# Stalfoes/dqn_mgsc_zoo

Hardware: AMD Instinct MI355X
Metric: learner grad-steps/sec at batch=32, 84×84×4 uint8, 1/2/4/8 MI355X (higher is better)
Workload: dtype f32

## Files before the change

dqn_mgsc_zoo_amd/_native.py:

```python

import ctypes
import glob
import hashlib
import os
import threading

_HERE = os.path.dirname(os.path.abspath(__file__))
LIB_PATH = os.environ.get('DQZ_LIB') or os.path.join(_HERE, 'libdqz.so')
HEADER_PATH = os.path.join(os.path.dirname(_HERE), 'include', 'dqz.h')

DQZ_OK = 0
ALGO_DQN = 0
ALGO_DOUBLE = 1
ALGO_PER = 2
NUM_LEAVES = 10
NUM_PHASES = 10
PHASE_NAMES = (
    'conv1_fwd', 'conv2_fwd', 'conv3_fwd', 'fc1_fwd', 'head', 'fc1_dx',
    'conv3_dx+conv2_dx+fc1_dw+conv3_dw+conv2_dw+conv1_dw', 'unused7',
    'unused8', 'update')
FRAME_H = 84
FRAME_W = 84
STACK = 4
FRAME_BYTES = FRAME_H * FRAME_W
# ... 272 lines not shown
    'dqz_qr_forward_slots': (
        _int, [_vp, _vp, ctypes.POINTER(DqzStore), _vp, _int, _int, _vp, _vp]),
    'dqz_qr_act': (
        _int, [_vp, _vp, _vp, _int, ctypes.c_double, ctypes.c_uint64,
               ctypes.c_uint64, _vp, _vp]),
    'dqz_qr_debug_check': (_int, [_int, ctypes.c_uint]),
    'dqz_learner_grad': (
        _int,
        [_vp, ctypes.POINTER(DqzParams), ctypes.POINTER(DqzStore), _vp, _vp,
         _vp, _vp],
    ),
    'dqz_learner_outputs': (_int, [_vp, _vp, _vp, _vp, _vp]),
    'dqz_learner_sync_status': (_int, [_vp, _vp]),
    'dqz_learner_debug_stall': (_int, [_vp, _int, ctypes.c_uint]),
    'dqz_learner_debug_backward': (_int, [_vp, _int, _vp]),
    'dqz_learner_debug_activations': (_int, [_vp, _int] + [_vp] * 10),
    'dqz_per_write_back': (_int, [_vp, _vp, _i64, _vp, ctypes.c_double, _vp, _vp]),
    'dqz_learner_profile': (
        _int,
        [_vp, ctypes.POINTER(DqzParams), ctypes.POINTER(DqzStore), _vp, _vp,
         _int, ctypes.POINTER(ctypes.c_float), _vp],
    ),
    'dqz_forward': (_int, [_vp, _vp, _vp, _int, _vp, _vp]),
    'dqz_forward_slots': (
        _int, [_vp, _vp, ctypes.POINTER(DqzStore), _vp, _int, _int, _vp, _vp]),
    'dqz_act': (
        _int, [_vp, _vp, _vp, _int, ctypes.c_double, ctypes.c_uint64,
               ctypes.c_uint64, _vp, _vp]),
    'dqz_store_put': (
        _int, [ctypes.POINTER(DqzStore), ctypes.POINTER(DqzTransitionPut), _vp,
# ... 159 lines not shown
```

dqn_mgsc_zoo_amd/csrc/bwd.hpp:

```cpp
#pragma once
#include "common.hpp"
#include "conv1.hpp"
#include "fwd.hpp"
#include "head.hpp"
#include "sampling.hpp"

namespace dqz {

struct Fc1BwdArgs {
  const float* dz1;
  const float* y3;
  float *th, *mu, *nu;
  int64_t w_off;
  Rms rms;
  int B;
  float* dy3;
  const float *w3, *w2;
  float *w3p, *w2p;
};

__device__ __forceinline__ int w3p_src(int i) {
  const int j = i & 3, kq = (i >> 2) & 3, n = (i >> 4) & 15, w = (i >> 8) & 3, r = i >> 10;
  const int tp = r % 9, nq = r / 9;
  return ((8 - tp) * C3CI + 16 * nq + n) * C3CO + 16 * w + 4 * j + kq;
// ... 296 lines not shown
      const float4 v = wp[tp * 256];
      wr[4 * tp] = v.x;
      wr[4 * tp + 1] = v.y;
      wr[4 * tp + 2] = v.z;
      wr[4 * tp + 3] = v.w;
    }
#pragma unroll
    for (int k = 0; k < 2; ++k) {
      const int q = min((t >> 2) + 64 * k, 99), ah = q / 10, cw = q % 10;
      ym4[k] = *reinterpret_cast<const float4*>(a.y1 + ((int64_t)b * C1M + (2 * ah + ph) * C1O + 2 * cw + pw) * C1CO +
                                                16 * hh + 4 * (t & 3));
    }
  }
  const float4* src = reinterpret_cast<const float4*>(a.dy2 + (int64_t)b * (C2M * C2CO));
  constexpr int NW4 = 121 * 16;
  if constexpr (WAIT) a.sync.wait(b);
  float4 r[8];
#pragma unroll
  for (int q = 0; q < 8; ++q) {
    const int i = min(t + 256 * q, NW4 - 1);
    const int pix = i >> 4, oh = pix / 11 - 1, ow = pix % 11 - 1;
    const bool in = oh >= 0 && oh < C2O && ow >= 0 && ow < C2O;
    const int e = (in ? oh * C2O + ow : 0) * 16 + (i & 15);
    float4 v;
    if constexpr (WAIT)
      v = load_sc1_f4(src, C2M * C2CO * 4, e);
    else
      v = src[e];
    r[q] = in ? v : make_float4(0.f, 0.f, 0.f, 0.f);
  }
  __builtin_amdgcn_sched_barrier(0);
#pragma unroll
  for (int q = 0; q < 8; ++q) {
    const int i = t + 256 * q;
    if (i < NW4) {
      const int pix = i >> 4;
      float* d = s_win + (pix / 11) * C2X_RS + (pix % 11) * C2X_S + win64_ch((i & 15) * 4);
      d[0] = r[q].x;
      d[1] = r[q].y;
      d[2] = r[q].z;
      d[3] = r[q].w;
    }
  }
  __syncthreads();
  DQZ_STAMP(7, 1);
  constexpr int MT = 6;
  int base[MT];
#pragma unroll
  for (int m = 0; m < MT; ++m) {
    const int p = min(16 * m + n, 99);
    base[m] = (p / 10) * C2X_RS + (p % 10) * C2X_S + win64_ch(16 * w) + kq;
  }
  f32x4 acc[MT];
#pragma unroll
  for (int m = 0; m < MT; ++m) acc[m] = f32x4{0.f, 0.f, 0.f, 0.f};
  float last[4] = {0.f, 0.f, 0.f, 0.f};
#pragma unroll
  for (int kk = 0; kk < 16; ++kk) {
    const int tp = kk >> 2;
// ... 1 lines not shown
#pragma unroll
    for (int m = 0; m < MT; ++m) acc[m] = mfma4(s_win[base[m] + off], wr[kk], acc[m]);
    {
#pragma unroll
      for (int e = 0; e < 4; ++e)
        last[e] = __fmaf_rn(s_win[9 * C2X_RS + (6 + e) * C2X_S + win64_ch(16 * w) + kq + off], wr[kk], last[e]);
    }
  }
  {
#pragma unroll
    for (int e = 0; e < 4; ++e) {
      last[e] += __shfl_xor(last[e], 16, 64);
      last[e] += __shfl_xor(last[e], 32, 64);
    }
  }
  __syncthreads();
  DQZ_STAMP(7, 2);
  float* s_red = s_win;
#pragma unroll
  for (int m = 0; m < MT; ++m)
#pragma unroll
    for (int rr = 0; rr < 4; ++rr) s_red[w * 1792 + (16 * m + 4 * kq + rr) * 16 + n] = acc[m][rr];
  if (kq == 0) {
#pragma unroll
    for (int e = 0; e < 4; ++e) s_red[w * 1792 + (96 + e) * 16 + n] = last[e];
  }
  __syncthreads();
#pragma unroll
  for (int k = 0; k < 2; ++k) {
    const int q = (t >> 2) + 64 * k;
// ... 4 lines not shown
      for (int e = 0; e < 4; ++e)
        v[e] = (s_red[i + e] + s_red[1792 + i + e]) + (s_red[3584 + i + e] + s_red[5376 + i + e]);
      v[0] = ym4[k].x > 0.f ? v[0] : 0.f;
      v[1] = ym4[k].y > 0.f ? v[1] : 0.f;
      v[2] = ym4[k].z > 0.f ? v[2] : 0.f;
      v[3] = ym4[k].w > 0.f ? v[3] : 0.f;
      float* slab = a.dy1 + (int64_t)b * C1M * C1CO;
      const int off = (((2 * ah + ph) * C1O + 2 * cw + pw) * C1CO + 16 * hh + 4 * (t & 3)) * 4;
      if constexpr (PUB)
        store_sc1_f4(slab, C1M * C1CO * 4, off, v);
      else
        *reinterpret_cast<f32x4*>(reinterpret_cast<char*>(slab) + off) = v;
    }
  }
  if constexpr (PUB) a.sync1.arrive(b);
}

constexpr int C2V_WIN = 9 * C2W_RS;

__device__ __forceinline__ void conv2_bwd_dw_split(const Conv2BwdArgs& a, float* s_win, int b, int kh, int ch) {
  const int t = threadIdx.x, lane = t & 63, w = t >> 6;
  const int n = lane & 15, kq = lane >> 4;
  constexpr int NV4 = 9 * C1O * C1CO / 4;
  float4 r[6];
  {
    const float4* src = reinterpret_cast<const float4*>(a.y1 + (int64_t)b * (C1M * C1CO));
#pragma unroll
    for (int q = 0; q < 6; ++q) {
      const int i = min(t + 256 * q, NV4 - 1);
      const int oh = i / (C1O * 8), rem = i % (C1O * 8);
// ... 7 lines not shown
    pb[kk] = (p / C2O) * C2W_RS + (2 * (p % C2O) + w) * C2W_S + n;
  }
  f32x4 acc[2][2];
#pragma unroll
  for (int mt = 0; mt < 2; ++mt)
#pragma unroll
    for (int ct = 0; ct < 2; ++ct) acc[mt][ct] = f32x4{0.f, 0.f, 0.f, 0.f};
#pragma unroll
  for (int q = 0; q < 6; ++q) {
    const int i = t + 256 * q;
    if (i < NV4) {
      const int oh = i / (C1O * 8), rem = i % (C1O * 8), iw = rem >> 3;
      *reinterpret_cast<float4*>(s_win + oh * C2W_RS + iw * C2W_S + (rem & 7) * 4) = r[q];
    }
  }
  a.sync.wait(b);
  float dr[21][2];
#pragma unroll
  for (int kk = 0; kk < 21; ++kk) {
    const int p = 4 * kk + kq;
#pragma unroll
    for (int ct = 0; ct < 2; ++ct) {
      const float* gp = a.dy2 + ((int64_t)b * C2M + min(p, C2M - 1)) * C2CO + 32 * ch + 16 * ct + n;
      const float v = __hip_atomic_load(gp, __ATOMIC_RELAXED, __HIP_MEMORY_SCOPE_AGENT);
      dr[kk][ct] = p < C2M ? v : 0.f;
    }
  }
  __syncthreads();
  DQZ_STAMP(13, 1);
#pragma unroll
  for (int kk = 0; kk < 21; ++kk)
#pragma unroll
    for (int mt = 0; mt < 2; ++mt) {
      const float av = s_win[pb[kk] + 16 * mt];
#pragma unroll
      for (int ct = 0; ct < 2; ++ct) acc[mt][ct] = mfma4(dr[kk][ct], av, acc[mt][ct]);
    }
  float sb[2] = {0.f, 0.f};
#pragma unroll
  for (int ct = 0; ct < 2; ++ct)
#pragma unroll
    for (int kk = 0; kk < 21; ++kk) sb[ct] += dr[kk][ct];
  float* slab = a.part + (int64_t)b * (C2KK + 1) * C2CO;
#pragma unroll
  for (int mt = 0; mt < 2; ++mt)
#pragma unroll
    for (int ct = 0; ct < 2; ++ct)
      *reinterpret_cast<f32x4*>(slab + ((kh * C2K + w) * C2CI + 16 * mt + n) * C2CO + 32 * ch + 16 * ct + 4 * kq) =
          acc[mt][ct];
  if (kh == 0 && w == 0) {
#pragma unroll
    for (int ct = 0; ct < 2; ++ct) {
// ... 341 lines not shown
```

dqn_mgsc_zoo_amd/csrc/common.hpp:

```cpp
#pragma once
#include <hip/hip_runtime.h>

#include <cstdarg>
#include <cstdint>
#include <cstdio>
#include <string>

#include "dqz.h"

namespace dqz {

typedef float f32x4 __attribute__((ext_vector_type(4)));

#define DQZ_STR(x) #x
#define DQZ_XSTR(x) DQZ_STR(x)
typedef float f32x16 __attribute__((ext_vector_type(16)));

#ifdef DQZ_STEP_TU
#define DQZ_STEP_KERNEL __global__
#define DQZ_OTHER_KERNEL template <int = 0> __global__
#else
#define DQZ_STEP_KERNEL template <int = 0> __global__
#define DQZ_OTHER_KERNEL __global__
#endif
// ... 100 lines not shown
    const float w = 2.f * u * (-lr) * rs3 * (d2 - c1 * g * (g - m));
    nu = w;
    sq += u * u;
    s1 += gq * w;
  }
  __device__ __forceinline__ float meta2(float g, float m0, float v0, float j, float& sq) const {
    const float m = c1 * g + decay * m0;
    const float v = c1 * (g * g) + decay * v0;
    const float u = (-lr) * (g * rsqrtf(v - m * m + eps));
    sq += u * u;
    return -2.f * u * j;
  }
};

#ifdef DQZ_TRACE
constexpr int TRACE_KERNELS = 20, TRACE_BLOCKS = 4096, TRACE_SLOTS = 4;
static __device__ unsigned long long g_dqz_trace[TRACE_KERNELS * TRACE_BLOCKS * TRACE_SLOTS];
#define DQZ_STAMP(kid, slot)                                                                              \
  do {                                                                                                    \
    if (threadIdx.x == 0) {                                                                               \
      const unsigned bl_ = blockIdx.x + gridDim.x * (blockIdx.y + gridDim.y * blockIdx.z);                \
      if (bl_ < (unsigned)dqz::TRACE_BLOCKS)                                                              \
        dqz::g_dqz_trace[((kid) * dqz::TRACE_BLOCKS + bl_) * dqz::TRACE_SLOTS + (slot)] =                \
            __builtin_amdgcn_s_memrealtime();                                                             \
    }                                                                                                     \
  } while (0)
#else
#define DQZ_STAMP(kid, slot) \
  do {                       \
  } while (0)
#endif
// ... 71 lines not shown

inline dim3 xcd_grid(int J, int nsamp) { return dim3((unsigned)(J * ((nsamp + 7) / 8) * 8)); }

struct Handoff {
  static constexpr int kStride = 64;
  int* cnt;
  int* ack;
  int* err;
  int need, consumers;
  unsigned spin_max = 1u << 24;
  __device__ __forceinline__ void arrive(int b) const {
    asm volatile("s_waitcnt vmcnt(0)" ::: "memory");
    __syncthreads();
    if (threadIdx.x == 0) __hip_atomic_fetch_add(cnt + b * kStride, 1, __ATOMIC_RELAXED, __HIP_MEMORY_SCOPE_AGENT);
  }
  __device__ __forceinline__ void wait(int b) const {
    if (threadIdx.x == 0) {
      unsigned spins = 0;
      while (__hip_atomic_load(cnt + b * kStride, __ATOMIC_RELAXED, __HIP_MEMORY_SCOPE_AGENT) < need) {
        __builtin_amdgcn_s_sleep(4);
        if (++spins > spin_max) {
          __hip_atomic_fetch_or(err, 1, __ATOMIC_RELAXED, __HIP_MEMORY_SCOPE_AGENT);
          break;
        }
      }
      if (__hip_atomic_fetch_add(ack + b * kStride, 1, __ATOMIC_RELAXED, __HIP_MEMORY_SCOPE_AGENT) == consumers - 1) {
        __hip_atomic_store(cnt + b * kStride, 0, __ATOMIC_RELAXED, __HIP_MEMORY_SCOPE_AGENT);
        __hip_atomic_store(ack + b * kStride, 0, __ATOMIC_RELAXED, __HIP_MEMORY_SCOPE_AGENT);
      }
    }
    __syncthreads();
  }
};

__device__ __forceinline__ float4 load_sc1_f4(const float4* base, int bytes, int e) {
  typedef unsigned u32x4 __attribute__((ext_vector_type(4)));
  const __amdgpu_buffer_rsrc_t r = __builtin_amdgcn_make_buffer_rsrc((void*)base, 0, bytes, 0x00020000);
  return __builtin_bit_cast(float4, __builtin_amdgcn_raw_buffer_load_b128(r, e * 16, 0, 16));
}

__device__ __forceinline__ float load_sc1_f1(const float* base, int bytes, int e) {
  const __amdgpu_buffer_rsrc_t r = __builtin_amdgcn_make_buffer_rsrc((void*)base, 0, bytes, 0x00020000);
  return __builtin_bit_cast(float, __builtin_amdgcn_raw_buffer_load_b32(r, e * 4, 0, 16));
}

__device__ __forceinline__ void store_sc1_f4(float* base, int bytes, int off, f32x4 v) {
  typedef unsigned u32x4 __attribute__((ext_vector_type(4)));
  const __amdgpu_buffer_rsrc_t r = __builtin_amdgcn_make_buffer_rsrc((void*)base, 0, bytes, 0x00020000);
// ... 26 lines not shown
```

dqn_mgsc_zoo_amd/csrc/conv1.hpp:

```cpp
#pragma once
#include "common.hpp"
#include "sampling.hpp"

namespace dqz {

struct Conv1Src {
  const uint8_t* frames;
  const int32_t* fidx;
  const int32_t* slots;
  const uint8_t* states;
  int fused;
  union {
    UniformDraw draw;
    SoftmaxDraw sm;
    PerSampleArgs per;
    SoftmaxDrawExact smx;
  };
  const int32_t* action = nullptr;
  const float* reward = nullptr;
  const float* discount = nullptr;
  float4* rec = nullptr;
  uint8_t* xout = nullptr;
};

// ... 272 lines not shown
  const int row0 = rb * C1S * C1_ROWS;
  constexpr int QPC = C1_PLANE / 16;
  uint4 v = make_uint4(0u, 0u, 0u, 0u);
  const int tid = threadIdx.x;
  const int cl = tid / QPC, pj = tid % QPC;
  if constexpr (PRE) {
    v = vpre;
  } else {
    const int slot = a.src.slots[b];
    const int32_t* fr = a.src.fidx + (int64_t)slot * 8 + a.which * 4 + 2 * ch;
    const int fa = fr[0], fb = fr[1];
    const int f = cl == 0 ? fa : fb;
    if (tid < 2 * QPC && f >= 0)
      v = reinterpret_cast<const uint4*>(a.src.frames + (int64_t)f * FB + row0 * FW)[pj];
  }
  a.sync1.wait(b);
  const float* dyb = a.dy1 + ((int64_t)b * C1M + rb * C1_POS) * C1CO;
  const int co = tid & 31, c0 = tid >> 5;
  float dv[2][8];
#pragma unroll
  for (int it = 0; it < 2; ++it) {
    const int c = c0 + 8 * it, oh = c / 3, ow0 = 8 * (c % 3);
#pragma unroll
    for (int j = 0; j < 8; ++j)
      dv[it][j] = (c < 15 && ow0 + j < C1O)
                      ? load_sc1_f1(dyb, C1_POS * C1CO * 4, (oh * C1O + ow0 + j) * C1CO + co) : 0.f;
  }
  if (tid < 2 * QPC) store_bytes_as_bf16(s_in + cl * C1_PLANE + pj * 16, v);
#pragma unroll
  for (int it = 0; it < 2; ++it) {
    const int c = c0 + 8 * it;
    unsigned pk[3][4];
    float sb = 0.f;
#pragma unroll
    for (int j = 0; j < 8; j += 2) {
      unsigned h0, m0, l0, h1, m1, l1;
      split3_bf16(dv[it][j], h0, m0, l0);
      split3_bf16(dv[it][j + 1], h1, m1, l1);
      pk[0][j / 2] = h0 | (h1 << 16);
      pk[1][j / 2] = m0 | (m1 << 16);
      pk[2][j / 2] = l0 | (l1 << 16);
      sb += dv[it][j];
      sb += dv[it][j + 1];
    }
#pragma unroll
    for (int q = 0; q < 3; ++q)
      *reinterpret_cast<uint4*>(s_dt + (q * C1CO + co) * C1H_TLD + 8 * c) =
          make_uint4(pk[q][0], pk[q][1], pk[q][2], pk[q][3]);
    s_bp[c * C1CO + co] = sb;
  }
  __syncthreads();
  DQZ_STAMP(8, 1);
  const int lane = tid & 63, wave = tid >> 6;
  const int h = lane >> 5, i = lane & 31;
  float* part = a.part + ((int64_t)b * C1_BLOCKS + rb) * (C1KK + 1) * C1CO;
  if (ch == 0 && tid < C1CO) {
    float sb = 0.f;
    for (int c = 0; c < 15; ++c) sb += s_bp[c * C1CO + tid];
    part[C1KK * C1CO + tid] = sb;
  }
  const int kh = 2 * wave + (i >> 4), kw = (i >> 1) & 7, cp = i & 1;
  const uint16_t* pb = s_in + cp * C1_PLANE + kh * FW + kw;
  const uint16_t* pa = s_dt + i * C1H_TLD + 8 * h;
  f32x16 acc = {};
#pragma unroll
  for (int s = 0; s < 8; ++s) {
    constexpr int R = 4 * FW;
    const int o0 = (2 * s) / 3 * R + 32 * ((2 * s) % 3);
    const int o1 = 2 * s + 1 < 15 ? (2 * s + 1) / 3 * R + 32 * ((2 * s + 1) % 3) : 0;
    const uint16_t* px = pb + (h ? o1 : o0);
    unsigned xp[4];
#pragma unroll
    for (int j = 0; j < 8; j += 2) xp[j / 2] = (unsigned)px[4 * j] | ((unsigned)px[4 * j + 4] << 16);
    const bf16x8 xb = __builtin_bit_cast(bf16x8, make_uint4(xp[0], xp[1], xp[2], xp[3]));
#pragma unroll
    for (int q = 0; q < 3; ++q) {
      const bf16x8 dq = __builtin_bit_cast(bf16x8, *reinterpret_cast<const uint4*>(pa + q * C1CO * C1H_TLD + 16 * s));
      acc = __builtin_amdgcn_mfma_f32_32x32x16_bf16(dq, xb, acc, 0, 0, 0);
    }
  }
  {
    const int row = (2 * wave + (i >> 4)) * 32 + ((i >> 1) & 7) * 4 + 2 * ch + (i & 1);
#pragma unroll
    for (int q = 0; q < 4; ++q)
      *reinterpret_cast<f32x4*>(part + row * C1CO + 8 * q + 4 * h) =
          f32x4{div255(acc[4 * q]), div255(acc[4 * q + 1]), div255(acc[4 * q + 2]), div255(acc[4 * q + 3])};
  }
  DQZ_STAMP(8, 3);
}

__device__ __forceinline__ void conv1_dw_half(const Conv1DwArgs& a, float* smem, int rb, int ch, int b) {
  DQZ_STAMP(8, 0);
  conv1_dw_body<false>(a, smem, make_uint4(0u, 0u, 0u, 0u), rb, ch, b);
}

// ... 2 lines not shown
```

dqn_mgsc_zoo_amd/csrc/fwd.hpp:

```cpp
#pragma once
#include "common.hpp"
#include "conv1.hpp"

namespace dqz {


__device__ __forceinline__ f32x4 mfma4(float a, float b, f32x4 c) {
  return __builtin_amdgcn_mfma_f32_16x16x4f32(a, b, c, 0, 0, 0);
}

__device__ __forceinline__ int red_idx(int row, int col) { return row * 16 + 16 * (row >> 2) + col; }

__device__ __forceinline__ int epi_row(int i) {
  return ((i >> 6) << 4) + (int)((0xFBAE9DC873261540ull >> (4 * ((i >> 2) & 15))) & 15);
}
constexpr int epi_range(int rows) { return (rows + 15) / 16 * 64; }
constexpr int red_rows(int rows) { return rows * 16 + 16 * ((rows + 3) / 4); }

struct LayerFwdArgs {
  const float* in;
  NetZ nz;
  int64_t w_off, b_off;
  int B, Z;
  int linear;
// ... 8 lines not shown
template <bool WAIT, bool PUB>
__device__ __forceinline__ void conv2_fwd_body(const LayerFwdArgs& a, float* s_in, const SampleJob sj) {
  DQZ_STAMP(1, 0);
  const int nq = sj.job, b = sj.s % a.B, z = sj.s / a.B;
  const int t = threadIdx.x, lane = t & 63, w = t >> 6;
  const int n = lane & 15, kq = lane >> 4;
  const float* W = a.nz.p[z] + a.w_off;
  const float bv = a.nz.p[z][a.b_off + 16 * nq + (t & 15)];
  const float4 bias4 = PUB ? *reinterpret_cast<const float4*>(a.nz.p[z] + a.b_off + 16 * nq + 4 * (t & 3))
                           : make_float4(0.f, 0.f, 0.f, 0.f);
  float wr[32];
#pragma unroll
  for (int kk = 0; kk < 32; ++kk) wr[kk] = W[(w * 128 + 4 * kk + kq) * C2CO + 16 * nq + n];
  const float4* src = reinterpret_cast<const float4*>(a.in + ((int64_t)z * a.B + b) * (C1M * C1CO));
  constexpr int NQ4 = C1M * C1CO / 4;
  if constexpr (WAIT) a.wait.wait(sj.s);
  float4 r[13];
#pragma unroll
  for (int q = 0; q < 13; ++q) {
    if constexpr (WAIT)
      r[q] = load_sc1_f4(src, NQ4 * 16, min(t + 256 * q, NQ4 - 1));
    else
      r[q] = src[min(t + 256 * q, NQ4 - 1)];
  }
  __builtin_amdgcn_sched_barrier(0);
#pragma unroll
  for (int q = 0; q < 13; ++q) {
    const int i = t + 256 * q;
    if (i < NQ4) {
      const int pix = i >> 3, ci = (i & 7) * 4;
      float* d = s_in + (pix / C1O) * C2L_RS + (pix % C1O) * C2L_S + ci;
      d[0] = r[q].x;
      d[1] = r[q].y;
      d[2] = r[q].z;
      d[3] = r[q].w;
    }
  }
  DQZ_STAMP(1, 1);
  __syncthreads();
  constexpr int MT = 5;
  int base[MT];
#pragma unroll
  for (int m = 0; m < MT; ++m) {
    const int p = min(16 * m + n, C2M - 1);
    base[m] = (2 * (p / C2O) + w) * C2L_RS + 2 * (p % C2O) * C2L_S + kq;
  }
  f32x4 acc[MT];
#pragma unroll
  for (int m = 0; m < MT; ++m) acc[m] = f32x4{0.f, 0.f, 0.f, 0.f};
  float last = 0.f;
  const int blast = (2 * (C2O - 1) + w) * C2L_RS + 2 * (C2O - 1) * C2L_S + kq;
#pragma unroll
  for (int kk = 0; kk < 32; ++kk) {
    const int off = (kk >> 3) * C2L_S + 4 * (kk & 7);
#pragma unroll
    for (int m = 0; m < MT; ++m) acc[m] = mfma4(s_in[base[m] + off], wr[kk], acc[m]);
    last = __fmaf_rn(s_in[blast + off], wr[kk], last);
  }
  DQZ_STAMP(1, 2);
  {
    last += __shfl_xor(last, 16, 64);
    last += __shfl_xor(last, 32, 64);
  }
  __syncthreads();
  float* s_red = s_in;
  constexpr int RW = red_rows(96);
  static_assert(4 * RW <= C2L_WIN, "conv2 partials fit the window");
#pragma unroll
  for (int m = 0; m < MT; ++m)
#pragma unroll
    for (int rr = 0; rr < 4; ++rr) s_red[w * RW + red_idx(16 * m + 4 * kq + rr, n)] = acc[m][rr];
  if (kq == 0) s_red[w * RW + red_idx(C2M - 1, n)] = last;
  __syncthreads();
  float* out = a.out + ((int64_t)z * a.B + b) * (C2M * C2CO) + 16 * nq;
// ... 4 lines not shown
  if constexpr (PUB) {
    for (int i = t; i < epi_range(C2M); i += 256) {
      const int p = epi_row(i), c4 = 4 * (i & 3);
      if (p >= C2M) continue;
      float o[4];
#pragma unroll
      for (int e = 0; e < 4; ++e) {
        const int k = red_idx(p, c4 + e);
        const float bb = e == 0 ? bias4.x : e == 1 ? bias4.y : e == 2 ? bias4.z : bias4.w;
        const float v = ((s_red[k] + s_red[RW + k]) + (s_red[2 * RW + k] + s_red[3 * RW + k])) + bb;
        o[e] = linear ? v : relu(v);
      }
      store_sc1_f4(out, (C2M * C2CO - 16 * nq) * 4, 4 * (p * C2CO + c4), f32x4{o[0], o[1], o[2], o[3]});
    }
    a.pub.arrive(sj.s);
  } else {
    for (int i = t; i < C2M * 16; i += 256) {
      const int k = red_idx(i >> 4, i & 15);
      const float v = ((s_red[k] + s_red[RW + k]) + (s_red[2 * RW + k] + s_red[3 * RW + k])) + bv;
      if (dot)
        dacc += v * dyp[(i >> 4) * C2CO + (i & 15)];
      else
        out[(i >> 4) * C2CO + (i & 15)] = linear ? v : relu(v);
    }
  }
  if (!PUB && dot) {
    __syncthreads();
    const float r = block_sum256(dacc, s_in);
    if (t == 0) a.dot.part[(int64_t)b * META_DOT_SLOTS + a.dot.slot0 + nq] = r;
  }
// ... 4 lines not shown
__device__ __forceinline__ void conv2_fwd8_body(const LayerFwdArgs& a, float* s_in, const SampleJob sj) {
  DQZ_STAMP(1, 0);
  const int rh = sj.job >> 2, nq = sj.job & 3, b = sj.s % a.B, z = sj.s / a.B;
  const int oh0 = rh * C2F_ROWS0, npos = (rh ? C2O - C2F_ROWS0 : C2F_ROWS0) * C2O;
  const int ih0 = C2S * oh0, nrows = C2S * (npos / C2O - 1) + C2K;
  const int t = threadIdx.x, lane = t & 63, w = t >> 6;
  const int n = lane & 15, kq = lane >> 4;
  const float* W = a.nz.p[z] + a.w_off;
  const float4 bias4 = *reinterpret_cast<const float4*>(a.nz.p[z] + a.b_off + 16 * nq + 4 * (t & 3));
  float wr[32];
#pragma unroll
  for (int kk = 0; kk < 32; ++kk) wr[kk] = W[(w * 128 + 4 * kk + kq) * C2CO + 16 * nq + n];
  const float4* src = reinterpret_cast<const float4*>(a.in + ((int64_t)z * a.B + b) * (C1M * C1CO)) +
                      ih0 * C1O * (C1CO / 4);
  const int nq4 = nrows * C1O * (C1CO / 4);
  a.wait.wait(sj.s);
  constexpr int NL = (2 * C2F_ROWS0 + 2) * C1O * (C1CO / 4) / 256;
  float4 r[NL + 1];
#pragma unroll
  for (int q = 0; q <= NL; ++q) r[q] = load_sc1_f4(src, nq4 * 16, min(t + 256 * q, nq4 - 1));
  __builtin_amdgcn_sched_barrier(0);
#pragma unroll
  for (int q = 0; q <= NL; ++q) {
    const int i = t + 256 * q;
    if (i < nq4) {
      const int pix = i >> 3, ci = (i & 7) * 4;
      float* d = s_in + (pix / C1O) * C2L_RS + (pix % C1O) * C2L_S + ci;
      d[0] = r[q].x;
      d[1] = r[q].y;
      d[2] = r[q].z;
      d[3] = r[q].w;
    }
  }
  DQZ_STAMP(1, 1);
  __syncthreads();
  constexpr int MT = 3;
  int base[MT];
#pragma unroll
  for (int m = 0; m < MT; ++m) {
    const int p = min(16 * m + n, npos - 1);
    base[m] = (2 * (p / C2O) + w) * C2L_RS + 2 * (p % C2O) * C2L_S + kq;
  }
  f32x4 acc[MT];
#pragma unroll
  for (int m = 0; m < MT; ++m) acc[m] = f32x4{0.f, 0.f, 0.f, 0.f};
#pragma unroll
  for (int kk = 0; kk < 32; ++kk) {
    const int off = (kk >> 3) * C2L_S + 4 * (kk & 7);
#pragma unroll
    for (int m = 0; m < MT; ++m) acc[m] = mfma4(s_in[base[m] + off], wr[kk], acc[m]);
// ... 13 lines not shown
  const bool linear = a.linear;
  for (int i = t; i < epi_range(npos); i += 256) {
    const int p = epi_row(i), c4 = 4 * (i & 3);
    if (p >= npos) continue;
    float o[4];
#pragma unroll
    for (int e = 0; e < 4; ++e) {
      const int k = red_idx(p, c4 + e);
      const float bb = e == 0 ? bias4.x : e == 1 ? bias4.y : e == 2 ? bias4.z : bias4.w;
      const float v = ((s_red[k] + s_red[RW + k]) + (s_red[2 * RW + k] + s_red[3 * RW + k])) + bb;
      o[e] = linear ? v : relu(v);
    }
    store_sc1_f4(out, out_bytes, 4 * (p * C2CO + c4), f32x4{o[0], o[1], o[2], o[3]});
  }
  a.pub.arrive(sj.s);
  DQZ_STAMP(1, 3);
}


constexpr int C3L_S = 66, C3L_RS = 622, C3L_WIN = 9 * C3L_RS;

template <bool WAIT>
__device__ __forceinline__ void conv3_fwd_body(const LayerFwdArgs& a, float* s_in, const SampleJob sj) {
  DQZ_STAMP(2, 0);
  const int nq = sj.job, b = sj.s % a.B, z = sj.s / a.B;
  const int t = threadIdx.x, lane = t & 63, w = t >> 6;
  const int n = lane & 15, kq = lane >> 4;
  const float* W = a.nz.p[z] + a.w_off;
  const float bv = a.nz.p[z][a.b_off + 16 * nq + (t & 15)];
  float wr[36];
#pragma unroll
  for (int kk = 0; kk < 36; ++kk)
    wr[kk] = W[((kk >> 2) * C3CI + 16 * w + 4 * (kk & 3) + kq) * C3CO + 16 * nq + n];
  const float4* src = reinterpret_cast<const float4*>(a.in + ((int64_t)z * a.B + b) * (C2M * C2CO));
  constexpr int NQ4 = C2M * C2CO / 4;
  if constexpr (WAIT) a.wait.wait(sj.s);
  float4 r[6];
#pragma unroll
  for (int q = 0; q < 6; ++q) {
    if constexpr (WAIT)
      r[q] = load_sc1_f4(src, NQ4 * 16, min(t + 256 * q, NQ4 - 1));
    else
      r[q] = src[min(t + 256 * q, NQ4 - 1)];
  }
  __builtin_amdgcn_sched_barrier(0);
#pragma unroll
  for (int q = 0; q < 6; ++q) {
    const int i = t + 256 * q;
    if (i < NQ4) {
      const int pix = i >> 4, ci = (i & 15) * 4;
      float* d = s_in + (pix / C2O) * C3L_RS + (pix % C2O) * C3L_S + win64_ch(ci);
      d[0] = r[q].x;
      d[1] = r[q].y;
      d[2] = r[q].z;
      d[3] = r[q].w;
    }
  }
  DQZ_STAMP(2, 1);
  __syncthreads();
  constexpr int MT = 3;
  int base[MT];
#pragma unroll
  for (int m = 0; m < MT; ++m) {
    const int p = min(16 * m + n, C3M - 1);
    base[m] = (p / C3O) * C3L_RS + (p % C3O) * C3L_S + win64_ch(16 * w) + kq;
  }
  f32x4 acc[MT];
#pragma unroll
  for (int m = 0; m < MT; ++m) acc[m] = f32x4{0.f, 0.f, 0.f, 0.f};
  float last = 0.f;
  const int blast = (C3O - 1) * C3L_RS + (C3O - 1) * C3L_S + win64_ch(16 * w) + kq;
#pragma unroll
  for (int kk = 0; kk < 36; ++kk) {
    const int tap = kk >> 2;
    const int off = (tap / 3) * C3L_RS + (tap % 3) * C3L_S + 4 * (kk & 3);
#pragma unroll
    for (int m = 0; m < MT; ++m) acc[m] = mfma4(s_in[base[m] + off], wr[kk], acc[m]);
    last = __fmaf_rn(s_in[blast + off], wr[kk], last);
  }
  DQZ_STAMP(2, 2);
  {
    last += __shfl_xor(last, 16, 64);
    last += __shfl_xor(last, 32, 64);
  }
  __syncthreads();
  float* s_red = s_in;
  constexpr int RW = red_rows(64);
  static_assert(4 * RW <= C3L_WIN, "conv3 partials fit the window");
#pragma unroll
  for (int m = 0; m < MT; ++m)
#pragma unroll
    for (int rr = 0; rr < 4; ++rr) s_red[w * RW + red_idx(16 * m + 4 * kq + rr, n)] = acc[m][rr];
  if (kq == 0) s_red[w * RW + red_idx(C3M - 1, n)] = last;
  __syncthreads();
  float* out = a.out + ((int64_t)z * a.B + b) * FLAT + 16 * nq;
// ... 24 lines not shown
  DQZ_STAMP(2, 0);
  const int rh = sj.job >> 2, nq = sj.job & 3, b = sj.s % a.B, z = sj.s / a.B;
  const int oh0 = rh * C3F_ROWS0, npos = (rh ? C3O - C3F_ROWS0 : C3F_ROWS0) * C3O;
  const int nrows = npos / C3O + C3K - 1;
  const int t = threadIdx.x, lane = t & 63, w = t >> 6;
  const int n = lane & 15, kq = lane >> 4;
  const float* W = a.nz.p[z] + a.w_off;
  const float4 bias4 = *reinterpret_cast<const float4*>(a.nz.p[z] + a.b_off + 16 * nq + 4 * (t & 3));
  float wr[36];
#pragma unroll
  for (int kk = 0; kk < 36; ++kk)
    wr[kk] = W[((kk >> 2) * C3CI + 16 * w + 4 * (kk & 3) + kq) * C3CO + 16 * nq + n];
  const float4* src = reinterpret_cast<const float4*>(a.in + ((int64_t)z * a.B + b) * (C2M * C2CO)) +
                      oh0 * C2O * (C2CO / 4);
  const int nq4 = nrows * C2O * (C2CO / 4);
  a.wait.wait(sj.s);
  constexpr int NL = ((C3F_ROWS0 + C3K - 1) * C2O * (C2CO / 4) + 255) / 256;
  float4 r[NL];
#pragma unroll
  for (int q = 0; q < NL; ++q) r[q] = load_sc1_f4(src, nq4 * 16, min(t + 256 * q, nq4 - 1));
  __builtin_amdgcn_sched_barrier(0);
#pragma unroll
  for (int q = 0; q < NL; ++q) {
    const int i = t + 256 * q;
    if (i < nq4) {
      const int pix = i >> 4, ci = (i & 15) * 4;
      float* d = s_in + (pix / C2O) * C3L_RS + (pix % C2O) * C3L_S + win64_ch(ci);
      d[0] = r[q].x;
      d[1] = r[q].y;
      d[2] = r[q].z;
      d[3] = r[q].w;
    }
  }
  DQZ_STAMP(2, 1);
  __syncthreads();
  constexpr int MT = 2;
  int base[MT];
#pragma unroll
  for (int m = 0; m < MT; ++m) {
    const int p = min(16 * m + n, npos - 1);
    base[m] = (p / C3O) * C3L_RS + (p % C3O) * C3L_S + win64_ch(16 * w) + kq;
  }
  f32x4 acc[MT];
#pragma unroll
  for (int m = 0; m < MT; ++m) acc[m] = f32x4{0.f, 0.f, 0.f, 0.f};
#pragma unroll
  for (int kk = 0; kk < 36; ++kk) {
    const int tap = kk >> 2;
    const int off = (tap / 3) * C3L_RS + (tap % 3) * C3L_S + 4 * (kk & 3);
#pragma unroll
    for (int m = 0; m < MT; ++m) acc[m] = mfma4(s_in[base[m] + off], wr[kk], acc[m]);
  }
  DQZ_STAMP(2, 2);
  __syncthreads();
  float* s_red = s_in;
  constexpr int RW = red_rows(16 * MT);
  static_assert(4 * RW <= C3L_WIN, "conv3 partials fit the window");
#pragma unroll
  for (int m = 0; m < MT; ++m)
#pragma unroll
    for (int rr = 0; rr < 4; ++rr) s_red[w * RW + red_idx(16 * m + 4 * kq + rr, n)] = acc[m][rr];
  __syncthreads();
  float* out = a.out + ((int64_t)z * a.B + b) * FLAT + oh0 * C3O * C3CO + 16 * nq;
  const bool linear = a.linear;
  for (int i = t; i < epi_range(npos); i += 256) {
    const int p = epi_row(i), c4 = 4 * (i & 3);
    if (p >= npos) continue;
    float o[4];
// ... 180 lines not shown
```

dqn_mgsc_zoo_amd/csrc/hvp.hpp:

```cpp
#pragma once
#include "common.hpp"

namespace dqz {

struct HvpArgs {
  const uint8_t* x;
  const float4* rec;
  const float* th;
  const float* tw;
  int64_t off[10];
  int A;
  const float *y1, *y2, *y3, *h;
  const float *d1, *d2, *d3, *d4;
  float *ty1, *ty2, *ty3, *td4, *td3, *td2, *td1;
  float* hq;
  float* part;
  const float* s1_part;
  int s1_nparts;
  float* s1;
  const float *vdir, *J, *gq, *td;
  float bound;
  float* vout;
  Handoff td1_pub;
};
// ... 517 lines not shown
    else
      *reinterpret_cast<float4*>(a.hq + a.off[6] + e[u]) = hq;
  }
}

__device__ __forceinline__ void hvp_g_conv1(const HvpArgs& a, int k, float (*s_r)[64], float* s_x, const HqOut& ho) {
  const int t = threadIdx.x, co = t & 31, sp = t >> 5;
  if (k < C1KK) {
    const int kh = k / (C1K * FC), kw = (k / FC) % C1K, ci = k % FC;
    const uint8_t* fr = a.x + ci * FB;
    for (int p = t; p < C1M; p += 256) s_x[p] = u8n(fr[(C1S * (p / C1O) + kh) * FW + C1S * (p % C1O) + kw]);
  } else {
    for (int p = t; p < C1M; p += 256) s_x[p] = 1.f;
  }
  DQZ_STAMP(18, 1);
  a.td1_pub.wait(0);
  DQZ_STAMP(18, 2);
  float tv[50];
#pragma unroll
  for (int j = 0; j < 50; ++j) tv[j] = load_sc1_f1(a.td1, C1M * C1CO * 4, (50 * sp + j) * C1CO + co);
  float g = 0.f;
#pragma unroll
  for (int j = 0; j < 50; ++j) g += s_x[50 * sp + j] * tv[j];
  s_r[sp][co] = g;
  __syncthreads();
  if (t < C1CO) {
    float v = 0.f;
#pragma unroll
    for (int s = 0; s < 8; ++s) v += s_r[s][t];
    ho.put(a, a.off[0] + (int64_t)k * C1CO + t, v);
  }
// ... 31 lines not shown
```

dqn_mgsc_zoo_amd/csrc/learner_step.hip:

```cpp
#define DQZ_STEP_TU 1
#include <hip/hip_runtime.h>

#include <cstdlib>
#include <cstring>

#include "learner_impl.hpp"

using namespace dqz;

static int g_attr_done = 0;

static int init_kernel_attrs() {
  if (g_attr_done) return DQZ_OK;
  const void* fwd_kernels[] = {(const void*)fwd_conv_kernel<0>, (const void*)fwd_conv_kernel<1>,
                               (const void*)fwd_conv_kernel<2>, (const void*)fwd_conv_kernel<3>,
                               (const void*)fwd_conv_kernel<4>};
  for (const void* k : fwd_kernels)
    DQZ_HIP(hipFuncSetAttribute(k, hipFuncAttributeMaxDynamicSharedMemorySize, (int)kConv1FwdSmem));
  g_attr_done = 1;
  return DQZ_OK;
}

extern "C" {

// ... 414 lines not shown
    const SyncLayout at = sync_of(L);
    DQZ_HIP(hipDeviceSynchronize());
    DQZ_HIP(hipMemcpy(L->sync + at.dy2().cnt + at.word(sample), &poison, sizeof(poison), hipMemcpyHostToDevice));
  }
  return DQZ_OK;
}

int dqz_learner_debug_backward(dqz_learner* L, int chain, int* active) {
  if (!L) return fail(DQZ_ERR_INVALID, "null learner");
  if (chain < -1 || chain > 1) return fail(DQZ_ERR_INVALID, "chain must be -1, 0 or 1");
  L->bwd_chain = chain;
  if (active) *active = bwd_chain_active(L) ? 1 : 0;
  return DQZ_OK;
}

int dqz_learner_outputs(dqz_learner* L, float* q_tm1, float* td, float* loss, void* stream) {
  if (!L) return fail(DQZ_ERR_INVALID, "null learner");
  hipStream_t st = (hipStream_t)stream;
  const int B = L->cfg.batch, A = L->cfg.num_actions;
  if (q_tm1) DQZ_HIP(hipMemcpyAsync(q_tm1, L->q, sizeof(float) * B * A, hipMemcpyDeviceToDevice, st));
  if (td) DQZ_HIP(hipMemcpyAsync(td, L->td, sizeof(float) * B, hipMemcpyDeviceToDevice, st));
  if (loss) DQZ_HIP(hipMemcpyAsync(loss, L->loss, sizeof(float), hipMemcpyDeviceToDevice, st));
  return DQZ_OK;
}

static int forward_q(dqz_learner* L, const float* params, const Conv1Src& src, int which, int n, float* q_out,
                     const ActorDraw* act, hipStream_t st) {
  if (int rc = forward_torso(L, params, src, which, n, st)) return rc;
  HeadArgs h = make_head(L, NetZ{{params, params, params}, {which, which, which}}, 1, n);
  h.fwd_only = 1;
// ... 50 lines not shown
```

dqn_mgsc_zoo_amd/learner.py:

```python

import ctypes

import numpy as np
import torch

from dqn_mgsc_zoo_amd import _native
from dqn_mgsc_zoo_amd import networks as networks_lib
from dqn_mgsc_zoo_amd import optim_state

ALGOS = {'dqn': _native.ALGO_DQN, 'double': _native.ALGO_DOUBLE,
         'per': _native.ALGO_PER}


class RMSPropConfig:

  def __init__(self, learning_rate, decay=0.9, eps=1e-8, centered=False):
    self.learning_rate = float(learning_rate)
    self.decay = float(decay)
    self.eps = float(eps)
    self.centered = bool(centered)


def rmsprop(learning_rate, decay=0.9, eps=1e-8, centered=False):
  return RMSPropConfig(learning_rate, decay, eps, centered)
# ... 313 lines not shown
    return self.q_tm1, self.td, self.loss

  def sync_status(self):
    st = ctypes.c_int(0)
    _native.check(_native.lib().dqz_learner_sync_status(self._h, ctypes.byref(st)))
    return st.value

  def debug_stall(self, sample, spin_max=0):
    _native.check(_native.lib().dqz_learner_debug_stall(self._h, int(sample), int(spin_max)))

  def debug_backward(self, chain=-1):
    active = ctypes.c_int(-1)
    _native.check(_native.lib().dqz_learner_debug_backward(
        self._h, int(chain), ctypes.byref(active)))
    return active.value

  def fetch_activations(self, z=0, backward=False, stream=None):
    b, a = self.batch_size, self.network.num_actions
    shapes = dict(y1=(b, 20, 20, 32), y2=(b, 9, 9, 64), y3=(b, 7, 7, 64),
                  h1=(b, 512), q=(b, a))
    if backward:
      shapes.update(dz1=(b, 512), dy3=(b, 7, 7, 64), dy2=(b, 9, 9, 64),
                    dy1=(b, 20, 20, 32))
    out = {k: torch.empty(s, dtype=torch.float32, device=self.device)
           for k, s in shapes.items()}
    _native.check(_native.lib().dqz_learner_debug_activations(
        self._h, int(z),
        *(_native.ptr(out.get(k)) for k in ('y1', 'y2', 'y3', 'h1', 'q', 'dz1',
                                             'dy3', 'dy2', 'dy1')),
        _native.stream_handle(stream)))
# ... 435 lines not shown
```

include/dqz.h:

```cpp
#ifndef DQZ_H_
#define DQZ_H_

#include <stdint.h>

#ifdef __cplusplus
extern "C" {
#endif

#define DQZ_OK 0
#define DQZ_ERR_INVALID (-1)
#define DQZ_ERR_HIP (-2)
#define DQZ_ERR_UNSUPPORTED (-3)

#define DQZ_ALGO_DQN 0
#define DQZ_ALGO_DOUBLE 1
#define DQZ_ALGO_PER 2

#define DQZ_FRAME_H 84
#define DQZ_FRAME_W 84
#define DQZ_STACK 4
#define DQZ_FRAME_BYTES (DQZ_FRAME_H * DQZ_FRAME_W)
#define DQZ_NUM_LEAVES 10

const char* dqz_last_error(void);
// ... 60 lines not shown
                     const int32_t* slots, const float* is_weights, float* grad_out, void* stream);

#define DQZ_NUM_PHASES 10

int dqz_learner_profile(dqz_learner* learner, const dqz_params* params, const dqz_store* store,
                        const int32_t* slots, const float* is_weights, int iters, float* phase_ms,
                        void* stream);

int dqz_learner_outputs(dqz_learner* learner, float* q_tm1, float* td, float* loss, void* stream);

int dqz_learner_sync_status(dqz_learner* learner, int* status);

int dqz_learner_debug_stall(dqz_learner* learner, int sample, unsigned spin_max);

int dqz_learner_debug_backward(dqz_learner* learner, int chain, int* active);

int dqz_learner_debug_activations(dqz_learner* learner, int z, float* y1, float* y2, float* y3, float* h1,
                                  float* q, float* dz1, float* dy3, float* dy2, float* dy1, void* stream);

int dqz_forward(dqz_learner* learner, const float* params, const uint8_t* states, int n,
                float* q_out, void* stream);

int dqz_forward_slots(dqz_learner* learner, const float* params, const dqz_store* store,
                      const int32_t* slots, int n, int which, float* q_out, void* stream);

typedef struct dqz_action {
  int32_t action;
  float value;
} dqz_action;
int dqz_act(dqz_learner* learner, const float* params, const uint8_t* states, int n, double epsilon,
// ... 289 lines not shown
```

Before: 16560.

## Split consumer ack out of sync wait and overlap it with compute

The cross-block sync wait no longer performs the serialized ack fetch-add and counter reset before its barrier. Consumers now issue the ack atomic after staging their input into shared memory and finish the reset later, after the MFMA loop, so the atomic's round-trip latency overlaps with compute instead of sitting on the critical path. Trace stamps and a debug entry point for reading the sync words are added. The ack address is offset by an mbcnt lane term that is zero for thread 0, so semantics stay the same but the reset point moves later, which lengthens the window before the counter can be reused.

Measured after the change: 16790 (median of 6 runs). 1.4% higher.

```diff
diff --git a/dqn_mgsc_zoo_amd/_native.py b/dqn_mgsc_zoo_amd/_native.py
--- a/dqn_mgsc_zoo_amd/_native.py
+++ b/dqn_mgsc_zoo_amd/_native.py
@@ -310,6 +310,7 @@
     'dqz_learner_sync_status': (_int, [_vp, _vp]),
     'dqz_learner_debug_stall': (_int, [_vp, _int, ctypes.c_uint]),
     'dqz_learner_debug_backward': (_int, [_vp, _int, _vp]),
+    'dqz_learner_debug_sync_words': (_int, [_vp, _vp, _i64, _vp]),
     'dqz_learner_debug_activations': (_int, [_vp, _int] + [_vp] * 10),
     'dqz_per_write_back': (_int, [_vp, _vp, _i64, _vp, ctypes.c_double, _vp, _vp]),
     'dqz_learner_profile': (
diff --git a/dqn_mgsc_zoo_amd/csrc/bwd.hpp b/dqn_mgsc_zoo_amd/csrc/bwd.hpp
--- a/dqn_mgsc_zoo_amd/csrc/bwd.hpp
+++ b/dqn_mgsc_zoo_amd/csrc/bwd.hpp
@@ -334,7 +334,7 @@
   }
   const float4* src = reinterpret_cast<const float4*>(a.dy2 + (int64_t)b * (C2M * C2CO));
   constexpr int NW4 = 121 * 16;
-  if constexpr (WAIT) a.sync.wait(b);
+  if constexpr (WAIT) a.sync.wait(b, kTraceDy2);
   float4 r[8];
 #pragma unroll
   for (int q = 0; q < 8; ++q) {
@@ -350,6 +350,7 @@
     r[q] = in ? v : make_float4(0.f, 0.f, 0.f, 0.f);
   }
   __builtin_amdgcn_sched_barrier(0);
+  if constexpr (WAIT) DQZ_STAMP(kTraceDy2, 2);
 #pragma unroll
   for (int q = 0; q < 8; ++q) {
     const int i = t + 256 * q;
@@ -363,6 +364,8 @@
     }
   }
   __syncthreads();
+  int ack = 0;
+  if constexpr (WAIT) ack = a.sync.release_issue(b);
   DQZ_STAMP(7, 1);
   constexpr int MT = 6;
   int base[MT];
@@ -394,6 +397,7 @@
       last[e] += __shfl_xor(last[e], 32, 64);
     }
   }
+  if constexpr (WAIT && !PUB) a.sync.release_finish(b, ack, kTraceDy2);
   __syncthreads();
   DQZ_STAMP(7, 2);
   float* s_red = s_win;
@@ -428,6 +432,7 @@
     }
   }
   if constexpr (PUB) a.sync1.arrive(b);
+  if constexpr (WAIT && PUB) a.sync.release_finish(b, ack, kTraceDy2);
 }
 
 constexpr int C2V_WIN = 9 * C2W_RS;
@@ -465,7 +470,7 @@
       *reinterpret_cast<float4*>(s_win + oh * C2W_RS + iw * C2W_S + (rem & 7) * 4) = r[q];
     }
   }
-  a.sync.wait(b);
+  a.sync.wait(b, kTraceDy2);
   float dr[21][2];
 #pragma unroll
   for (int kk = 0; kk < 21; ++kk) {
@@ -477,7 +482,9 @@
       dr[kk][ct] = p < C2M ? v : 0.f;
     }
   }
+  DQZ_STAMP(kTraceDy2, 2);
   __syncthreads();
+  const int ack = a.sync.release_issue(b);
   DQZ_STAMP(13, 1);
 #pragma unroll
   for (int kk = 0; kk < 21; ++kk)
@@ -487,6 +494,7 @@
 #pragma unroll
       for (int ct = 0; ct < 2; ++ct) acc[mt][ct] = mfma4(dr[kk][ct], av, acc[mt][ct]);
     }
+  a.sync.release_finish(b, ack, kTraceDy2);
   float sb[2] = {0.f, 0.f};
 #pragma unroll
   for (int ct = 0; ct < 2; ++ct)
diff --git a/dqn_mgsc_zoo_amd/csrc/common.hpp b/dqn_mgsc_zoo_amd/csrc/common.hpp
--- a/dqn_mgsc_zoo_amd/csrc/common.hpp
+++ b/dqn_mgsc_zoo_amd/csrc/common.hpp
@@ -138,7 +138,7 @@
 };
 
 #ifdef DQZ_TRACE
-constexpr int TRACE_KERNELS = 20, TRACE_BLOCKS = 4096, TRACE_SLOTS = 4;
+constexpr int TRACE_KERNELS = 24, TRACE_BLOCKS = 4096, TRACE_SLOTS = 4;
 static __device__ unsigned long long g_dqz_trace[TRACE_KERNELS * TRACE_BLOCKS * TRACE_SLOTS];
 #define DQZ_STAMP(kid, slot)                                                                              \
   do {                                                                                                    \
@@ -240,7 +240,7 @@
     __syncthreads();
     if (threadIdx.x == 0) __hip_atomic_fetch_add(cnt + b * kStride, 1, __ATOMIC_RELAXED, __HIP_MEMORY_SCOPE_AGENT);
   }
-  __device__ __forceinline__ void wait(int b) const {
+  __device__ __forceinline__ void wait(int b, [[maybe_unused]] int hk = -1) const {
     if (threadIdx.x == 0) {
       unsigned spins = 0;
       while (__hip_atomic_load(cnt + b * kStride, __ATOMIC_RELAXED, __HIP_MEMORY_SCOPE_AGENT) < need) {
@@ -250,14 +250,34 @@
           break;
         }
       }
-      if (__hip_atomic_fetch_add(ack + b * kStride, 1, __ATOMIC_RELAXED, __HIP_MEMORY_SCOPE_AGENT) == consumers - 1) {
-        __hip_atomic_store(cnt + b * kStride, 0, __ATOMIC_RELAXED, __HIP_MEMORY_SCOPE_AGENT);
-        __hip_atomic_store(ack + b * kStride, 0, __ATOMIC_RELAXED, __HIP_MEMORY_SCOPE_AGENT);
-      }
     }
+    if (hk >= 0) DQZ_STAMP(hk, 0);
     __syncthreads();
-  }
-};
+    if (hk >= 0) DQZ_STAMP(hk, 1);
+  }
+  __device__ __forceinline__ int release_issue(int b) const {
+    int prior = 0;
+    if (threadIdx.x == 0) {
+      int* p = ack + b * kStride + __builtin_amdgcn_mbcnt_lo(~0u, 0u);
+      prior = __hip_atomic_fetch_add(p, 1, __ATOMIC_RELAXED, __HIP_MEMORY_SCOPE_AGENT);
+    }
+    return prior;
+  }
+  __device__ __forceinline__ void release_finish(int b, int prior, [[maybe_unused]] int hk = -1) const {
+    __builtin_amdgcn_sched_barrier(0);
+    if (threadIdx.x == 0 && prior == consumers - 1) {
+      __hip_atomic_store(cnt + b * kStride, 0, __ATOMIC_RELAXED, __HIP_MEMORY_SCOPE_AGENT);
+      __hip_atomic_store(ack + b * kStride, 0, __ATOMIC_RELAXED, __HIP_MEMORY_SCOPE_AGENT);
+    }
+    if (hk >= 0) DQZ_STAMP(hk, 3);
+  }
+  __device__ __forceinline__ void wait_release(int b) const {
+    wait(b);
+    release_finish(b, release_issue(b));
+  }
+};
+
+constexpr int kTraceY1 = 20, kTraceY2 = 21, kTraceDy2 = 22, kTraceDy1 = 23;
 
 __device__ __forceinline__ float4 load_sc1_f4(const float4* base, int bytes, int e) {
   typedef unsigned u32x4 __attribute__((ext_vector_type(4)));
diff --git a/dqn_mgsc_zoo_amd/csrc/conv1.hpp b/dqn_mgsc_zoo_amd/csrc/conv1.hpp
--- a/dqn_mgsc_zoo_amd/csrc/conv1.hpp
+++ b/dqn_mgsc_zoo_amd/csrc/conv1.hpp
@@ -310,7 +310,7 @@
     if (tid < 2 * QPC && f >= 0)
       v = reinterpret_cast<const uint4*>(a.src.frames + (int64_t)f * FB + row0 * FW)[pj];
   }
-  a.sync1.wait(b);
+  a.sync1.wait(b, kTraceDy1);
   const float* dyb = a.dy1 + ((int64_t)b * C1M + rb * C1_POS) * C1CO;
   const int co = tid & 31, c0 = tid >> 5;
   float dv[2][8];
@@ -322,6 +322,7 @@
       dv[it][j] = (c < 15 && ow0 + j < C1O)
                       ? load_sc1_f1(dyb, C1_POS * C1CO * 4, (oh * C1O + ow0 + j) * C1CO + co) : 0.f;
   }
+  DQZ_STAMP(kTraceDy1, 2);
   if (tid < 2 * QPC) store_bytes_as_bf16(s_in + cl * C1_PLANE + pj * 16, v);
 #pragma unroll
   for (int it = 0; it < 2; ++it) {
@@ -346,6 +347,7 @@
     s_bp[c * C1CO + co] = sb;
   }
   __syncthreads();
+  const int ack = a.sync1.release_issue(b);
   DQZ_STAMP(8, 1);
   const int lane = tid & 63, wave = tid >> 6;
   const int h = lane >> 5, i = lane & 31;
@@ -375,6 +377,7 @@
       acc = __builtin_amdgcn_mfma_f32_32x32x16_bf16(dq, xb, acc, 0, 0, 0);
     }
   }
+  a.sync1.release_finish(b, ack, kTraceDy1);
   {
     const int row = (2 * wave + (i >> 4)) * 32 + ((i >> 1) & 7) * 4 + 2 * ch + (i & 1);
 #pragma unroll
diff --git a/dqn_mgsc_zoo_amd/csrc/fwd.hpp b/dqn_mgsc_zoo_amd/csrc/fwd.hpp
--- a/dqn_mgsc_zoo_amd/csrc/fwd.hpp
+++ b/dqn_mgsc_zoo_amd/csrc/fwd.hpp
@@ -46,7 +46,7 @@
   for (int kk = 0; kk < 32; ++kk) wr[kk] = W[(w * 128 + 4 * kk + kq) * C2CO + 16 * nq + n];
   const float4* src = reinterpret_cast<const float4*>(a.in + ((int64_t)z * a.B + b) * (C1M * C1CO));
   constexpr int NQ4 = C1M * C1CO / 4;
-  if constexpr (WAIT) a.wait.wait(sj.s);
+  if constexpr (WAIT) a.wait.wait(sj.s, kTraceY1);
   float4 r[13];
 #pragma unroll
   for (int q = 0; q < 13; ++q) {
@@ -56,6 +56,7 @@
       r[q] = src[min(t + 256 * q, NQ4 - 1)];
   }
   __builtin_amdgcn_sched_barrier(0);
+  if constexpr (WAIT) DQZ_STAMP(kTraceY1, 2);
 #pragma unroll
   for (int q = 0; q < 13; ++q) {
     const int i = t + 256 * q;
@@ -70,6 +71,8 @@
   }
   DQZ_STAMP(1, 1);
   __syncthreads();
+  int ack = 0;
+  if constexpr (WAIT) ack = a.wait.release_issue(sj.s);
   constexpr int MT = 5;
   int base[MT];
 #pragma unroll
@@ -90,6 +93,7 @@
     last = __fmaf_rn(s_in[blast + off], wr[kk], last);
   }
   DQZ_STAMP(1, 2);
+  if constexpr (WAIT && !PUB) a.wait.release_finish(sj.s, ack, kTraceY1);
   {
     last += __shfl_xor(last, 16, 64);
     last += __shfl_xor(last, 32, 64);
@@ -124,6 +128,7 @@
       store_sc1_f4(out, (C2M * C2CO - 16 * nq) * 4, 4 * (p * C2CO + c4), f32x4{o[0], o[1], o[2], o[3]});
     }
     a.pub.arrive(sj.s);
+    if constexpr (WAIT) a.wait.release_finish(sj.s, ack, kTraceY1);
   } else {
     for (int i = t; i < C2M * 16; i += 256) {
       const int k = red_idx(i >> 4, i & 15);
@@ -158,12 +163,13 @@
   const float4* src = reinterpret_cast<const float4*>(a.in + ((int64_t)z * a.B + b) * (C1M * C1CO)) +
                       ih0 * C1O * (C1CO / 4);
   const int nq4 = nrows * C1O * (C1CO / 4);
-  a.wait.wait(sj.s);
+  a.wait.wait(sj.s, kTraceY1);
   constexpr int NL = (2 * C2F_ROWS0 + 2) * C1O * (C1CO / 4) / 256;
   float4 r[NL + 1];
 #pragma unroll
   for (int q = 0; q <= NL; ++q) r[q] = load_sc1_f4(src, nq4 * 16, min(t + 256 * q, nq4 - 1));
   __builtin_amdgcn_sched_barrier(0);
+  DQZ_STAMP(kTraceY1, 2);
 #pragma unroll
   for (int q = 0; q <= NL; ++q) {
     const int i = t + 256 * q;
@@ -178,6 +184,7 @@
   }
   DQZ_STAMP(1, 1);
   __syncthreads();
+  const int ack = a.wait.release_issue(sj.s);
   constexpr int MT = 3;
   int base[MT];
 #pragma unroll
@@ -221,6 +228,7 @@
     store_sc1_f4(out, out_bytes, 4 * (p * C2CO + c4), f32x4{o[0], o[1], o[2], o[3]});
   }
   a.pub.arrive(sj.s);
+  a.wait.release_finish(sj.s, ack, kTraceY1);
   DQZ_STAMP(1, 3);
 }
 
@@ -241,7 +249,7 @@
     wr[kk] = W[((kk >> 2) * C3CI + 16 * w + 4 * (kk & 3) + kq) * C3CO + 16 * nq + n];
   const float4* src = reinterpret_cast<const float4*>(a.in + ((int64_t)z * a.B + b) * (C2M * C2CO));
   constexpr int NQ4 = C2M * C2CO / 4;
-  if constexpr (WAIT) a.wait.wait(sj.s);
+  if constexpr (WAIT) a.wait.wait(sj.s, kTraceY2);
   float4 r[6];
 #pragma unroll
   for (int q = 0; q < 6; ++q) {
@@ -251,6 +259,7 @@
       r[q] = src[min(t + 256 * q, NQ4 - 1)];
   }
   __builtin_amdgcn_sched_barrier(0);
+  if constexpr (WAIT) DQZ_STAMP(kTraceY2, 2);
 #pragma unroll
   for (int q = 0; q < 6; ++q) {
     const int i = t + 256 * q;
@@ -265,6 +274,8 @@
   }
   DQZ_STAMP(2, 1);
   __syncthreads();
+  int ack = 0;
+  if constexpr (WAIT) ack = a.wait.release_issue(sj.s);
   constexpr int MT = 3;
   int base[MT];
 #pragma unroll
@@ -286,6 +297,7 @@
     last = __fmaf_rn(s_in[blast + off], wr[kk], last);
   }
   DQZ_STAMP(2, 2);
+  if constexpr (WAIT) a.wait.release_finish(sj.s, ack, kTraceY2);
   {
     last += __shfl_xor(last, 16, 64);
     last += __shfl_xor(last, 32, 64);
@@ -340,12 +352,13 @@
   const float4* src = reinterpret_cast<const float4*>(a.in + ((int64_t)z * a.B + b) * (C2M * C2CO)) +
                       oh0 * C2O * (C2CO / 4);
   const int nq4 = nrows * C2O * (C2CO / 4);
-  a.wait.wait(sj.s);
+  a.wait.wait(sj.s, kTraceY2);
   constexpr int NL = ((C3F_ROWS0 + C3K - 1) * C2O * (C2CO / 4) + 255) / 256;
   float4 r[NL];
 #pragma unroll
   for (int q = 0; q < NL; ++q) r[q] = load_sc1_f4(src, nq4 * 16, min(t + 256 * q, nq4 - 1));
   __builtin_amdgcn_sched_barrier(0);
+  DQZ_STAMP(kTraceY2, 2);
 #pragma unroll
   for (int q = 0; q < NL; ++q) {
     const int i = t + 256 * q;
@@ -360,6 +373,7 @@
   }
   DQZ_STAMP(2, 1);
   __syncthreads();
+  const int ack = a.wait.release_issue(sj.s);
   constexpr int MT = 2;
   int base[MT];
 #pragma unroll
@@ -378,6 +392,7 @@
     for (int m = 0; m < MT; ++m) acc[m] = mfma4(s_in[base[m] + off], wr[kk], acc[m]);
   }
   DQZ_STAMP(2, 2);
+  a.wait.release_finish(sj.s, ack, kTraceY2);
   __syncthreads();
   float* s_red = s_in;
   constexpr int RW = red_rows(16 * MT);
diff --git a/dqn_mgsc_zoo_amd/csrc/hvp.hpp b/dqn_mgsc_zoo_amd/csrc/hvp.hpp
--- a/dqn_mgsc_zoo_amd/csrc/hvp.hpp
+++ b/dqn_mgsc_zoo_amd/csrc/hvp.hpp
@@ -555,7 +555,7 @@
     for (int p = t; p < C1M; p += 256) s_x[p] = 1.f;
   }
   DQZ_STAMP(18, 1);
-  a.td1_pub.wait(0);
+  a.td1_pub.wait_release(0);
   DQZ_STAMP(18, 2);
   float tv[50];
 #pragma unroll
diff --git a/dqn_mgsc_zoo_amd/csrc/learner_step.hip b/dqn_mgsc_zoo_amd/csrc/learner_step.hip
--- a/dqn_mgsc_zoo_amd/csrc/learner_step.hip
+++ b/dqn_mgsc_zoo_amd/csrc/learner_step.hip
@@ -452,6 +452,18 @@
   return DQZ_OK;
 }
 
+int dqz_learner_debug_sync_words(dqz_learner* L, int32_t* out, int64_t n, int64_t* total) {
+  if (!L) return fail(DQZ_ERR_INVALID, "null learner");
+  const int64_t ints = sync_of(L).ints();
+  if (total) *total = ints;
+  if (n < 0 || n > ints) return fail(DQZ_ERR_INVALID, "n must be in [0, %lld]", (long long)ints);
+  if (n > 0 && !out) return fail(DQZ_ERR_INVALID, "null out");
+  if (n == 0) return DQZ_OK;
+  DQZ_HIP(hipDeviceSynchronize());
+  DQZ_HIP(hipMemcpy(out, L->sync, sizeof(int32_t) * n, hipMemcpyDeviceToHost));
+  return DQZ_OK;
+}
+
 int dqz_learner_outputs(dqz_learner* L, float* q_tm1, float* td, float* loss, void* stream) {
   if (!L) return fail(DQZ_ERR_INVALID, "null learner");
   hipStream_t st = (hipStream_t)stream;
diff --git a/dqn_mgsc_zoo_amd/learner.py b/dqn_mgsc_zoo_amd/learner.py
--- a/dqn_mgsc_zoo_amd/learner.py
+++ b/dqn_mgsc_zoo_amd/learner.py
@@ -351,6 +351,14 @@
     _native.check(_native.lib().dqz_learner_debug_backward(
         self._h, int(chain), ctypes.byref(active)))
     return active.value
+
+  def debug_sync_words(self):
+    total = ctypes.c_int64(0)
+    fn = _native.lib().dqz_learner_debug_sync_words
+    _native.check(fn(self._h, None, 0, ctypes.byref(total)))
+    out = np.zeros((total.value,), np.int32)
+    _native.check(fn(self._h, out.ctypes.data, total.value, None))
+    return out
 
   def fetch_activations(self, z=0, backward=False, stream=None):
     b, a = self.batch_size, self.network.num_actions
diff --git a/include/dqz.h b/include/dqz.h
--- a/include/dqz.h
+++ b/include/dqz.h
@@ -98,6 +98,8 @@
 int dqz_learner_debug_stall(dqz_learner* learner, int sample, unsigned spin_max);
 
 int dqz_learner_debug_backward(dqz_learner* learner, int chain, int* active);
+
+int dqz_learner_debug_sync_words(dqz_learner* learner, int32_t* out, int64_t n, int64_t* total);
 
 int dqz_learner_debug_activations(dqz_learner* learner, int z, float* y1, float* y2, float* y3, float* h1,
                                   float* q, float* dz1, float* dy3, float* dy2, float* dy1, void* stream);
```
